# intel/hexl

Measured on NVIDIA H100. Metric: ntt_per_sec_fwd_inv_N65536_q55_batch8192, higher is better.
Workload: dtype u64

## Files before the change

hexl_b200/csrc/ntt_kernels.cuh:

```cuda
#pragma once
#include <algorithm>
#include <atomic>
#include <cstdio>
#include <cstdlib>

#include "internal.h"

namespace hexl_b200 {
namespace {

template <int I>
struct Idx {
  __host__ __device__ constexpr operator int() const { return I; }
};
template <int BEGIN, int END, typename F>
__device__ __forceinline__ void static_for(F&& f) {
  if constexpr (BEGIN < END) {
    f(Idx<BEGIN>{});
    static_for<BEGIN + 1, END>(f);
  }
}

enum : int { kGeneric = 0, kFast = 1, kSmall = 2, kWide = 3 };

template <int MODE>
struct Ar {
  using E = u64;
  using Tw = Twiddle;
};
template <>
struct Ar<kSmall> {
  using E = unsigned;
  using Tw = Twiddle32;
};
constexpr u64 kFastModulusLimit = 1ull << 56;
constexpr u64 kWideModulusLimit = 1ull << 61;
constexpr int kFastProd = 4;
constexpr int kFastBound = 8;

struct Mod {
  u64 q, two_q, four_q, mu;
  unsigned n0, n1;
};

__device__ __forceinline__ unsigned lo32(u64 x) { return (unsigned)x; }
__device__ __forceinline__ unsigned hi32(u64 x) { return (unsigned)(x >> 32); }
__device__ __forceinline__ u64 join(unsigned lo, unsigned hi) {
  u64 r;
  asm("mov.b64 %0, {%1, %2};" : "=l"(r) : "r"(lo), "r"(hi));
  return r;
}
__device__ __forceinline__ void split(u64 x, unsigned& lo, unsigned& hi) {
  asm("mov.b64 {%0, %1}, %2;" : "=r"(lo), "=r"(hi) : "l"(x));
}
__device__ __forceinline__ u64 mul_wide(unsigned a, unsigned b) {
  u64 r;
  asm("mul.wide.u32 %0, %1, %2;" : "=l"(r) : "r"(a), "r"(b));
  return r;
}
__device__ __forceinline__ u64 mad_wide(unsigned a, unsigned b, u64 c) {
  u64 r;
  asm("mad.wide.u32 %0, %1, %2, %3;" : "=l"(r) : "r"(a), "r"(b), "l"(c));
  return r;
}
__device__ __forceinline__ unsigned mad_lo(unsigned a, unsigned b, unsigned c) {
  unsigned r;
  asm("mad.lo.u32 %0, %1, %2, %3;" : "=r"(r) : "r"(a), "r"(b), "r"(c));
  return r;
}

__device__ __forceinline__ Twiddle ld_tw(const Twiddle* p) {
  const ulonglong2 v = __ldg(reinterpret_cast<const ulonglong2*>(p));
  Twiddle t;
  t.w = v.x;
  t.wp = v.y;
  return t;
}
__device__ __forceinline__ Twiddle32 ld_tw(const Twiddle32* p) {
  const uint2 v = __ldg(reinterpret_cast<const uint2*>(p));
  Twiddle32 t;
  t.w = v.x;
  t.wp = v.y;
  return t;
}

__device__ __forceinline__ u64 mulhi_approx(u64 a, u64 b) {
  unsigned a0, a1, b0, b1;
  split(a, a0, a1);
  split(b, b0, b1);
  const u64 hs = (u64)hi32(mul_wide(a1, b0)) + (u64)hi32(mul_wide(a0, b1));
  return mad_wide(a1, b1, hs);
}

__device__ __forceinline__ u64 mad_chain(u64 x, u64 w, u64 Q, const Mod& m) {
  unsigned x0, x1, w0, w1, q0, q1, t0, t1;
  split(x, x0, x1);
  split(w, w0, w1);
  split(Q, q0, q1);
  split(mad_wide(q0, m.n0, mul_wide(x0, w0)), t0, t1);
  t1 = mad_lo(x0, w1, t1);
  t1 = mad_lo(x1, w0, t1);
  t1 = mad_lo(q0, m.n1, t1);
  t1 = mad_lo(q1, m.n0, t1);
  return join(t0, t1);
}

template <int MODE>
__device__ __forceinline__ u64 mul_tw(u64 x, const Twiddle w, const Mod& m) {
  const u64 Q = (MODE == kFast || MODE == kWide) ? mulhi_approx(x, w.wp) : mulhi(x, w.wp);
  return mad_chain(x, w.w, Q, m);
}
__device__ __forceinline__ u64 mul_tw_exact(u64 x, const Twiddle w, const Mod& m) {
  return mad_chain(x, w.w, mulhi(x, w.wp), m);
}

__device__ __forceinline__ u64 barrett_lazy(u64 x, const Mod& m) {
  unsigned q0, q1, t0, t1;
  split(mulhi(x, m.mu), q0, q1);
  split(mad_wide(q0, m.n0, x), t0, t1);
  t1 = mad_lo(q0, m.n1, t1);
  t1 = mad_lo(q1, m.n0, t1);
  return join(t0, t1);
}
__device__ __forceinline__ u64 barrett_lazy_bigq(u64 x, const Mod& m) {
  unsigned x0, x1, s0, s1, t0, t1, Q, dummy;
  split(x, x0, x1);
  const unsigned mu0 = lo32(m.mu);
  split(mul_wide(x1, mu0), s0, s1);
  const unsigned h = hi32(mul_wide(x0, mu0));
  asm("add.cc.u32 %0, %2, %3;\n\taddc.u32 %1, %4, 0;" : "=r"(dummy), "=r"(Q) : "r"(s0), "r"(h), "r"(s1));
  split(mad_wide(Q, m.n0, x), t0, t1);
  return join(t0, mad_lo(Q, m.n1, t1));
}
__device__ __forceinline__ u64 barrett_lazy3_bigq(u64 x, const Mod& m) {
  unsigned x0, x1, t0, t1;
  split(x, x0, x1);
  const unsigned Q = hi32(mul_wide(x1, lo32(m.mu)));
  split(mad_wide(Q, m.n0, x), t0, t1);
  return join(t0, mad_lo(Q, m.n1, t1));
}

__device__ __forceinline__ u64 reduce_any(u64 x, const Mod& m) { return csub_s(barrett_lazy(x, m), m.q); }
__device__ __forceinline__ unsigned reduce_any(unsigned x, const Mod& m) { return x % (unsigned)m.q; }

struct ProdIn {
  const u64* b;
  u64 mu;
  int shift;
};
template <int MODE>
__device__ __forceinline__ u64 prod_lazy(u64 x, u64 y, const Mod& m, u64 pmu, int shift) {
  unsigned x0, x1, y0, y1, q0, q1, t0, t1;
  split(x, x0, x1);
  split(y, y0, y1);
  const u64 t = mul_wide(x0, y0);
  const u64 uu = mad_wide(x0, y1, (u64)hi32(t));
  const u64 vv = mad_wide(x1, y0, (u64)lo32(uu));
  const u64 hi = mad_wide(x1, y1, (u64)hi32(uu) + (u64)hi32(vv));
  const u64 lo = join(lo32(t), lo32(vv));
  const u64 c1 = shift ? ((lo >> shift) | (hi << (64 - shift))) : lo;
  const u64 Q = (MODE == kFast || MODE == kWide) ? mulhi_approx(c1, pmu) : mulhi(c1, pmu);
  split(Q, q0, q1);
  split(mad_wide(q0, m.n0, lo), t0, t1);
  t1 = mad_lo(q0, m.n1, t1);
  t1 = mad_lo(q1, m.n0, t1);
  return join(t0, t1);
}

template <int MODE, typename TW>
__device__ __forceinline__ void fwd_bfly(u64& X, u64& Y, const TW& w, const Mod& m) {
  if (MODE == kFast) {
    const u64 T = mul_tw<kFast>(Y, w, m);
    Y = X + m.four_q - T;
    X = X + T;
  } else if (MODE == kWide) {
    const u64 tx = csub(X, m.four_q);
    const u64 T = mul_tw<kWide>(Y, w, m);
    X = tx + T;
    Y = tx + m.four_q - T;
  } else {
    const u64 tx = csub_s(X, m.two_q);
    const u64 T = mul_tw<kGeneric>(Y, w, m);
    X = tx + T;
    Y = tx + m.two_q - T;
  }
}

template <int MODE, typename TW>
__device__ __forceinline__ void inv_bfly(u64& X, u64& Y, const TW& w, const Mod& m, u64 cq) {
  if (MODE == kFast) {
    const u64 d = X + cq - Y;
    X = X + Y;
    Y = mul_tw<kFast>(d, w, m);
  } else if (MODE == kWide) {
    const u64 s = X + Y;
    const u64 d = X + m.four_q - Y;
    X = csub_s(s, m.four_q);
    Y = mul_tw<kWide>(d, w, m);
  } else {
    const u64 s = X + Y;
    const u64 d = X + m.two_q - Y;
    X = csub_s(s, m.two_q);
    Y = mul_tw<kGeneric>(d, w, m);
  }
}

__device__ __forceinline__ void inv_bfly_last(u64& X, u64& Y, const Twiddle inv_n, const Twiddle inv_n_w,
                                              const Mod& m, u64 cq) {
  const u64 s = X + Y;
  const u64 d = X + cq - Y;
  X = mul_tw_exact(s, inv_n, m);
  Y = mul_tw_exact(d, inv_n_w, m);
}

template <int MODE>
__device__ __forceinline__ u64 fwd_out(u64 v, const Mod& m, int out_mf) {
  if (MODE == kFast) {
    v = barrett_lazy_bigq(v, m);
    return out_mf == 1 ? csub_s(v, m.q) : v;
  }
  if (MODE == kWide) v = csub_s(v, m.four_q);
  return out_mf == 1 ? csub_s(csub_s(v, m.two_q), m.q) : v;
}
__device__ __forceinline__ u64 inv_out(u64 v, const Mod& m, int out_mf) {
  return out_mf == 1 ? csub_s(v, m.q) : v;
}

__device__ __forceinline__ unsigned csub32(unsigned x, unsigned c) { return min(x, x - c); }
__device__ __forceinline__ unsigned mul_tw32(unsigned x, const Twiddle32 w, const Mod& m) {
  const unsigned Q = hi32(mul_wide(x, w.wp));
  return mad_lo(Q, m.n0, x * w.w);
}
template <int MODE, typename TW>
__device__ __forceinline__ void fwd_bfly(unsigned& X, unsigned& Y, const TW& w, const Mod& m) {
  const unsigned two_q = lo32(m.two_q);
  const unsigned tx = csub32(X, two_q);
  const unsigned T = mul_tw32(Y, w, m);
  X = tx + T;
  Y = tx + two_q - T;
}
template <int MODE, typename TW>
__device__ __forceinline__ void inv_bfly(unsigned& X, unsigned& Y, const TW& w, const Mod& m, unsigned) {
  const unsigned two_q = lo32(m.two_q);
  const unsigned s = X + Y;
  const unsigned d = X + two_q - Y;
  X = csub32(s, two_q);
  Y = mul_tw32(d, w, m);
}
__device__ __forceinline__ void inv_bfly_last(unsigned& X, unsigned& Y, const Twiddle32 inv_n,
                                              const Twiddle32 inv_n_w, const Mod& m, unsigned) {
  const unsigned s = X + Y;
  const unsigned d = X + lo32(m.two_q) - Y;
  X = mul_tw32(s, inv_n, m);
  Y = mul_tw32(d, inv_n_w, m);
}
template <int MODE>
__device__ __forceinline__ unsigned fwd_out(unsigned v, const Mod& m, int out_mf) {
  return out_mf == 1 ? csub32(csub32(v, lo32(m.two_q)), lo32(m.q)) : v;
}
__device__ __forceinline__ unsigned inv_out(unsigned v, const Mod& m, int out_mf) {
  return out_mf == 1 ? csub32(v, lo32(m.q)) : v;
}

__host__ __device__ constexpr int inv_slot_bound(int K, int low) {
  if (low == 0) return kFastBound << K;
  int h = 0;
  for (int b = 0; b < K; ++b)
    if (low & (1 << b)) h = b;
  return kFastProd << (K - 1 - h);
}
__host__ __device__ constexpr int inv_stage_cover(int s) { return kFastBound << s; }
template <int MODE>
__device__ __forceinline__ typename Ar<MODE>::E stage_cq(int step, const Mod& m) {
  if (MODE == kFast) return (u64)inv_stage_cover(step) * m.q;
  if (MODE == kWide) return m.four_q;
  return (typename Ar<MODE>::E)m.two_q;
}

template <int K, int NSLOTS, int E = 0>
__device__ __forceinline__ void inv_pass_fixup(u64* v, const Mod& m) {
  if constexpr (E < NSLOTS) {
    if constexpr (inv_slot_bound(K, E & ((1 << K) - 1)) > kFastBound) v[E] = barrett_lazy3_bigq(v[E], m);
    inv_pass_fixup<K, NSLOTS, E + 1>(v, m);
  }
}

template <typename E>
__device__ __forceinline__ unsigned swz(unsigned j) {
  return j ^ ((j >> 4) & (sizeof(E) == 8 ? 15u : 31u));
}
__host__ __device__ constexpr unsigned pad_slot(int e, int lb) { return ((unsigned)e << lb) + (((unsigned)e << lb) >> 4); }
template <typename E>
__host__ __device__ constexpr unsigned row_elems(int logc) {
  return (1u << logc) + (sizeof(E) == 8 ? (1u << logc) >> 4 : 0u);
}

template <int LB>
__device__ __forceinline__ unsigned reg_index(unsigned u, int e) {
  return ((u >> LB) << (LB + 4)) | ((unsigned)e << LB) | (u & ((1u << LB) - 1u));
}

constexpr int kRowTwEntries = 17 * 16;
template <int LOGC, int LB, int HB, int LOB>
struct PassTw {
  static constexpr int kDepth = LOGC - LB - 4;
  static constexpr bool kShared = LOGC >= 8 && (HB - LOB) == 3 && (kDepth == 0 || kDepth == 4);
  static constexpr int kOffset = kDepth == 0 ? 0 : 16;
};

template <int LOGC, typename Tw>
__device__ __forceinline__ void load_row_twiddles(Tw* stab, unsigned tid, unsigned nthreads, u64 base,
                                                  const Tw* __restrict__ tw) {
  for (int idx = tid; idx < kRowTwEntries; idx += nthreads) {
    const int l = idx & 15;
    if (l == 0) continue;
    const u64 root = idx < 16 ? base : (base << 4) + ((idx - 16) >> 4);
    const int s = 31 - __clz(l);
    stab[idx] = ld_tw(tw + (root << s) + (l - (1 << s)));
  }
}

template <int MODE, int LOGC, int LB, int HB, int LOB, bool FWD>
__device__ __forceinline__ void reg_stages(typename Ar<MODE>::E (&v)[16], unsigned u, u64 base,
                                           const typename Ar<MODE>::Tw* __restrict__ tw,
                                           const typename Ar<MODE>::Tw* stab, const Mod& m, bool fold,
                                           typename Ar<MODE>::Tw inv_n, typename Ar<MODE>::Tw inv_n_w) {
  using PT = PassTw<LOGC, LB, HB, LOB>;
  using Tw = typename Ar<MODE>::Tw;
  const Tw* sroot = stab + PT::kOffset + ((u >> LB) << 4);
  static_for<0, HB - LOB + 1>([&](auto STEP) {
    constexpr int step = STEP;
    constexpr int beta = FWD ? HB - step : LOB + step;
    constexpr int eb = beta - LB;
    constexpr int sp = LOGC - 1 - beta;
    const typename Ar<MODE>::E cq = stage_cq<MODE>(step, m);
    auto fetch = [&](int g) {
      if constexpr (PT::kShared)
        return sroot[(8 >> eb) + g];
      else
        return ld_tw(tw + (base << (LOGC - 1 - beta)) + ((u64)(u >> LB) << (LB + 3 - beta)) + g);
    };
    auto groups = [&] {
      Tw wc[8 >> eb];
      if constexpr (FWD) static_for<0, (8 >> eb)>([&](auto G) { constexpr int g = G; wc[g] = fetch(g); });
      static_for<0, (8 >> eb)>([&](auto G) {
        constexpr int g = G;
        Tw wt;
        if constexpr (FWD)
          wt = wc[g];
        else
          wt = fetch(g);
        static_for<0, (1 << eb)>([&](auto L) {
          constexpr int e = (g << (eb + 1)) | L;
          if constexpr (FWD)
            fwd_bfly<MODE>(v[e], v[e | (1 << eb)], wt, m);
          else
            inv_bfly<MODE>(v[e], v[e | (1 << eb)], wt, m, cq);
        });
      });
    };
    if constexpr (!FWD && sp == 0) {
      if (fold) {
        static_for<0, (1 << eb)>([&](auto L) {
          constexpr int l = L;
          inv_bfly_last(v[l], v[l | (1 << eb)], inv_n, inv_n_w, m, cq);
        });
      } else {
        groups();
      }
    } else {
      groups();
    }
  });
  if constexpr (!FWD && MODE == kFast) {
    if (!(fold && LOGC - 1 - HB == 0)) inv_pass_fixup<HB - LOB + 1, 16>(v, m);
  }
}

template <int LB_FROM, int LB_TO, typename E>
__device__ __forceinline__ void smem_exchange(E (&v)[16], E* srow, unsigned u) {
  constexpr bool kWarpLocal = (LB_FROM > LB_TO ? LB_FROM : LB_TO) <= 5;
  if constexpr (sizeof(E) == 8) {
    const unsigned uf = reg_index<LB_FROM>(u, 0), ut = reg_index<LB_TO>(u, 0);
    E* wr = srow + (uf + (uf >> 4));
    const E* rd = srow + (ut + (ut >> 4));
    static_for<0, 16>([&](auto I) { constexpr int e = I; wr[pad_slot(e, LB_FROM)] = v[e]; });
    if (kWarpLocal)
      __syncwarp();
    else
      __syncthreads();
    static_for<0, 16>([&](auto I) { constexpr int e = I; v[e] = rd[pad_slot(e, LB_TO)]; });
  } else {
    static_for<0, 16>([&](auto I) { constexpr int e = I; srow[swz<E>(reg_index<LB_FROM>(u, e))] = v[e]; });
    if (kWarpLocal)
      __syncwarp();
    else
      __syncthreads();
    static_for<0, 16>([&](auto I) { constexpr int e = I; v[e] = srow[swz<E>(reg_index<LB_TO>(u, e))]; });
  }
}

template <int MODE, int LOGC, int PASS>
__device__ __forceinline__ void fwd_passes(typename Ar<MODE>::E (&v)[16], typename Ar<MODE>::E* srow, unsigned u,
                                           u64 base, const typename Ar<MODE>::Tw* tw,
                                           const typename Ar<MODE>::Tw* stab, const Mod& m) {
  using Tw = typename Ar<MODE>::Tw;
  constexpr int PREV_LB = (LOGC - 4 * PASS) > 0 ? (LOGC - 4 * PASS) : 0;
  constexpr int HB = LOGC - 4 * PASS - 1;
  if constexpr (HB >= 0) {
    constexpr int LB = (HB - 3) > 0 ? (HB - 3) : 0;
    smem_exchange<PREV_LB, LB>(v, srow, u);
    reg_stages<MODE, LOGC, LB, HB, LB, true>(v, u, base, tw, stab, m, false, Tw{}, Tw{});
    fwd_passes<MODE, LOGC, PASS + 1>(v, srow, u, base, tw, stab, m);
  }
}

template <int MODE, int LOGC, int PASS>
__device__ __forceinline__ void inv_passes(typename Ar<MODE>::E (&v)[16], typename Ar<MODE>::E* srow, unsigned u,
                                           u64 base, const typename Ar<MODE>::Tw* tw,
                                           const typename Ar<MODE>::Tw* stab, const Mod& m, bool fold,
                                           typename Ar<MODE>::Tw inv_n, typename Ar<MODE>::Tw inv_n_w) {
  constexpr int HB = LOGC - 4 * PASS - 1;
  constexpr int LB = (HB - 3) > 0 ? (HB - 3) : 0;
  reg_stages<MODE, LOGC, LB, HB, LB, false>(v, u, base, tw, stab, m, fold, inv_n, inv_n_w);
  if constexpr (PASS > 0) {
    constexpr int NHB = LOGC - 4 * (PASS - 1) - 1;
    constexpr int NLB = (NHB - 3) > 0 ? (NHB - 3) : 0;
    smem_exchange<LB, NLB>(v, srow, u);
    inv_passes<MODE, LOGC, PASS - 1>(v, srow, u, base, tw, stab, m, fold, inv_n, inv_n_w);
  }
}

constexpr int kRowMinBlocks = 3;
constexpr int kRowMinBlocks512 = 2;
constexpr int kRowMinBlocksSmall = 4;
template <int LOGC, int MODE = kGeneric>
struct RowCfg {
  using E = typename Ar<MODE>::E;
  using Tw = typename Ar<MODE>::Tw;
  static constexpr int C = 1 << LOGC;
  static constexpr int T = C / 16;
  static constexpr int ROWS = T >= 256 ? 1 : 256 / T;
  static constexpr int THREADS = T * ROWS;
  static constexpr int PASSES = (LOGC + 3) / 4;
  static constexpr bool TW_TABLES = LOGC >= 8;
  static constexpr size_t ROW_BYTES = (size_t)row_elems<E>(LOGC) * sizeof(E) + (TW_TABLES ? kRowTwEntries * sizeof(Tw) : 0);
  static constexpr size_t SMEM = (size_t)ROWS * ROW_BYTES;
  static constexpr int MIN_BLOCKS = THREADS <= 256 ? (MODE == kSmall ? kRowMinBlocksSmall : kRowMinBlocks)
                                                   : (THREADS == 512 ? kRowMinBlocks512 : 1);
};

enum : int { kStream = 0, kViaL2 = 1, kSmemRow = 2, kSmemRowPad = 3 };
template <int POLICY>
__device__ __forceinline__ u64 ld_coef(const u64* p) {
  return POLICY == kViaL2 ? __ldcg(p) : __ldcs(p);
}
template <int POLICY>
__device__ __forceinline__ void st_coef(u64* p, u64 v) {
  if (POLICY == kViaL2)
    __stcg(p, v);
  else
    __stcs(p, v);
}

template <int POLICY, typename E>
__device__ __forceinline__ E ld_row(const void* base, unsigned idx) {
  if constexpr (POLICY == kSmemRow)
    return static_cast<const E*>(base)[idx];
  else if constexpr (POLICY == kSmemRowPad)
    return static_cast<const E*>(base)[idx + (idx >> 4)];
  else
    return (E)ld_coef<POLICY>(static_cast<const u64*>(base) + idx);
}
template <int POLICY, typename E>
__device__ __forceinline__ void st_row(void* base, unsigned idx, E v) {
  if constexpr (POLICY == kSmemRow)
    static_cast<E*>(base)[idx] = v;
  else if constexpr (POLICY == kSmemRowPad)
    static_cast<E*>(base)[idx + (idx >> 4)] = v;
  else
    st_coef<POLICY>(static_cast<u64*>(base) + idx, v);
}

struct MirrorList {
  u64* const* p;
  unsigned count;
  u64 off;
};

template <int MODE, int LOGC, int LD, int ST>
__device__ __forceinline__ void row_fwd_body(void* out, const void* in, typename Ar<MODE>::E* srow, unsigned u,
                                             u64 base, const typename Ar<MODE>::Tw* __restrict__ tw, const Mod& m,
                                             int out_mf, bool active, typename Ar<MODE>::Tw* cta_stab = nullptr,
                                             bool reduce_in = false) {
  using E = typename Ar<MODE>::E;
  using Tw = typename Ar<MODE>::Tw;
  E v[16];
  constexpr int LB0 = LOGC - 4;
  Tw* stab = cta_stab ? cta_stab : reinterpret_cast<Tw*>(srow + row_elems<E>(LOGC));
  static_for<0, 16>([&](auto I) { constexpr int e = I; v[e] = ld_row<LD, E>(in, reg_index<LB0>(u, e)); });
  if constexpr (LD < kSmemRow && sizeof(E) == 8) {
    if (reduce_in) {
      static_for<0, 16>([&](auto I) { constexpr int e = I; v[e] = reduce_any(v[e], m); });
    }
  }
  if constexpr (RowCfg<LOGC>::TW_TABLES) {
    if (cta_stab)
      load_row_twiddles<LOGC>(stab, threadIdx.x, blockDim.x, base, tw);
    else
      load_row_twiddles<LOGC>(stab, u, (1u << LOGC) / 16, base, tw);
    __syncthreads();
  }
  reg_stages<MODE, LOGC, LB0, LOGC - 1, LB0, true>(v, u, base, tw, stab, m, false, Tw{}, Tw{});
  fwd_passes<MODE, LOGC, 1>(v, srow, u, base, tw, stab, m);
  static_for<0, 16>([&](auto I) { constexpr int e = I; v[e] = fwd_out<MODE>(v[e], m, out_mf); });
  constexpr int LB_OUT = LB0 < 4 ? LB0 : 4;
  if constexpr (LOGC > 4) smem_exchange<0, LB_OUT>(v, srow, u);
  if (active) {
    static_for<0, 16>([&](auto I) { constexpr int e = I; st_row<ST, E>(out, reg_index<LB_OUT>(u, e), v[e]); });
  }
}

template <int MODE, int LOGC, int LD, int ST>
__device__ __forceinline__ void row_inv_body(void* out, const void* in, typename Ar<MODE>::E* srow, unsigned u,
                                             u64 base, const typename Ar<MODE>::Tw* __restrict__ tw, const Mod& m,
                                             int out_mf, bool fold, typename Ar<MODE>::Tw inv_n,
                                             typename Ar<MODE>::Tw inv_n_w, bool active,
                                             typename Ar<MODE>::Tw* cta_stab = nullptr, const MirrorList* mir = nullptr,
                                             const ProdIn* prod = nullptr) {
  using Cfg = RowCfg<LOGC>;
  using E = typename Ar<MODE>::E;
  using Tw = typename Ar<MODE>::Tw;
  E v[16];
  constexpr int LB0 = LOGC - 4;
  constexpr int LB_IN = LB0 < 4 ? LB0 : 4;
  Tw* stab = cta_stab ? cta_stab : reinterpret_cast<Tw*>(srow + row_elems<E>(LOGC));
  static_for<0, 16>([&](auto I) { constexpr int e = I; v[e] = ld_row<LD, E>(in, reg_index<LB_IN>(u, e)); });
  if constexpr (LD < kSmemRow && sizeof(E) == 8) {
    if (prod) {
      static_for<0, 16>([&](auto I) {
        constexpr int e = I;
        v[e] = prod_lazy<MODE>(v[e], ld_coef<LD>(prod->b + reg_index<LB_IN>(u, e)), m, prod->mu, prod->shift);
      });
    }
  }
  if constexpr (Cfg::TW_TABLES) {
    if (cta_stab)
      load_row_twiddles<LOGC>(stab, threadIdx.x, blockDim.x, base, tw);
    else
      load_row_twiddles<LOGC>(stab, u, (1u << LOGC) / 16, base, tw);
    __syncthreads();
  }
  if constexpr (LOGC > 4) smem_exchange<LB_IN, 0>(v, srow, u);
  inv_passes<MODE, LOGC, Cfg::PASSES - 1>(v, srow, u, base, tw, stab, m, fold, inv_n, inv_n_w);
  if (active) {
    static_for<0, 16>([&](auto I) {
      constexpr int e = I;
      st_row<ST, E>(out, reg_index<LB0>(u, e), fold ? inv_out(v[e], m, out_mf) : v[e]);
    });
    if (mir && fold) {
      for (unsigned p = 0; p < mir->count; ++p) {
        static_for<0, 16>([&](auto I) {
          constexpr int e = I;
          mir->p[p][mir->off + reg_index<LB0>(u, e)] = (u64)inv_out(v[e], m, out_mf);
        });
      }
    }
  }
}

template <int MODE, int LOGC>
__global__ void __launch_bounds__(RowCfg<LOGC, MODE>::THREADS, RowCfg<LOGC, MODE>::MIN_BLOCKS)
    ntt_row_fwd(u64* result, const u64* operand, const typename Ar<MODE>::Tw* __restrict__ tw, const Mod m,
                u64 total_rows, unsigned rows_per_poly, int out_mf) {
  using Cfg = RowCfg<LOGC, MODE>;
  extern __shared__ __align__(16) unsigned char smem[];
  const unsigned row_local = threadIdx.x / Cfg::T, u = threadIdx.x % Cfg::T;
  u64 row = (u64)blockIdx.x * Cfg::ROWS + row_local;
  const bool active = row < total_rows;
  if (!active) row = total_rows - 1;
  const u64 base = (u64)rows_per_poly + (row % rows_per_poly);
  typename Cfg::Tw* cta_stab = nullptr;
  if (MODE == kSmall && Cfg::ROWS > 1 && Cfg::TW_TABLES && rows_per_poly == 1)
    cta_stab = reinterpret_cast<typename Cfg::Tw*>(smem + (size_t)row_elems<typename Cfg::E>(LOGC) * sizeof(typename Cfg::E));
  row_fwd_body<MODE, LOGC, kStream, kStream>(
      result + row * Cfg::C, operand + row * Cfg::C,
      reinterpret_cast<typename Cfg::E*>(smem + (size_t)row_local * Cfg::ROW_BYTES), u, base, tw, m, out_mf, active,
      cta_stab);
}

template <int MODE, int LOGC>
__global__ void __launch_bounds__(RowCfg<LOGC, MODE>::THREADS, RowCfg<LOGC, MODE>::MIN_BLOCKS)
    ntt_row_inv(u64* result, const u64* operand, const typename Ar<MODE>::Tw* __restrict__ tw, const Mod m,
                u64 total_rows, unsigned rows_per_poly, int out_mf, int fold, typename Ar<MODE>::Tw inv_n,
                typename Ar<MODE>::Tw inv_n_w) {
  using Cfg = RowCfg<LOGC, MODE>;
  extern __shared__ __align__(16) unsigned char smem[];
  const unsigned row_local = threadIdx.x / Cfg::T, u = threadIdx.x % Cfg::T;
  u64 row = (u64)blockIdx.x * Cfg::ROWS + row_local;
  const bool active = row < total_rows;
  if (!active) row = total_rows - 1;
  const u64 base = (u64)rows_per_poly + (row % rows_per_poly);
  typename Cfg::Tw* cta_stab = nullptr;
  if (MODE == kSmall && Cfg::ROWS > 1 && Cfg::TW_TABLES && rows_per_poly == 1)
    cta_stab = reinterpret_cast<typename Cfg::Tw*>(smem + (size_t)row_elems<typename Cfg::E>(LOGC) * sizeof(typename Cfg::E));
  row_inv_body<MODE, LOGC, kStream, kStream>(
      result + row * Cfg::C, operand + row * Cfg::C,
      reinterpret_cast<typename Cfg::E*>(smem + (size_t)row_local * Cfg::ROW_BYTES), u, base, tw, m, out_mf,
      fold != 0, inv_n, inv_n_w, active, cta_stab);
}

template <int MODE, int LOGR, bool FWD>
__device__ __forceinline__ void col_stages(typename Ar<MODE>::E (&v)[1 << LOGR], const typename Ar<MODE>::Tw* stw,
                                           const Mod& m, bool root_fold, typename Ar<MODE>::Tw inv_n,
                                           typename Ar<MODE>::Tw inv_n_w) {
  using E = typename Ar<MODE>::E;
  using Tw = typename Ar<MODE>::Tw;
  constexpr int R = 1 << LOGR;
  static_for<0, LOGR>([&](auto STEP) {
    constexpr int step = STEP;
    constexpr int s = FWD ? step : LOGR - 1 - step;
    constexpr int eb = LOGR - 1 - s;
    const E cq = stage_cq<MODE>(step, m);
    auto groups = [&] {
      static_for<0, (1 << s)>([&](auto GI) {
        constexpr int gi = GI;
        const Tw w = stw[(1 << s) + gi];
        static_for<0, (1 << eb)>([&](auto L) {
          constexpr int e = (gi << (eb + 1)) | L;
          if constexpr (FWD)
            fwd_bfly<MODE>(v[e], v[e | (1 << eb)], w, m);
          else
            inv_bfly<MODE>(v[e], v[e | (1 << eb)], w, m, cq);
        });
      });
    };
    if constexpr (!FWD && s == 0) {
      if (root_fold) {
        static_for<0, (1 << eb)>([&](auto L) {
          constexpr int l = L;
          inv_bfly_last(v[l], v[l | (1 << eb)], inv_n, inv_n_w, m, cq);
        });
      } else {
        groups();
      }
    } else {
      groups();
    }
  });
  if constexpr (!FWD && MODE == kFast) {
    if (!root_fold) inv_pass_fixup<LOGR, R>(v, m);
  }
}

template <int MODE, int LOGR, bool FWD, int LD, int ST>
__device__ __forceinline__ void col_body(u64* result, const u64* operand, u64 off, int log_stride,
                                         const typename Ar<MODE>::Tw* stw, const Mod& m, int out_mf, bool root_fold,
                                         typename Ar<MODE>::Tw inv_n, typename Ar<MODE>::Tw inv_n_w,
                                         const MirrorList* mir = nullptr, bool reduce_in = false) {
  using E = typename Ar<MODE>::E;
  constexpr int R = 1 << LOGR;
  E v[R];
  static_for<0, R>([&](auto I) {
    constexpr int e = I;
    v[e] = (E)ld_coef<LD>(operand + off + ((u64)e << log_stride));
  });
  if constexpr (FWD && sizeof(E) == 8) {
    if (reduce_in) {
      static_for<0, R>([&](auto I) { constexpr int e = I; v[e] = reduce_any(v[e], m); });
    }
  }
  col_stages<MODE, LOGR, FWD>(v, stw, m, root_fold, inv_n, inv_n_w);
  const bool final_out = !FWD && root_fold;
  static_for<0, R>([&](auto I) {
    constexpr int e = I;
    st_coef<ST>(result + off + ((u64)e << log_stride), final_out ? inv_out(v[e], m, out_mf) : v[e]);
  });
  if (mir && final_out) {
    for (unsigned p = 0; p < mir->count; ++p) {
      static_for<0, R>([&](auto I) {
        constexpr int e = I;
        mir->p[p][mir->off + off + ((u64)e << log_stride)] = (u64)inv_out(v[e], m, out_mf);
      });
    }
  }
}

template <int MODE, int LOGR, bool FWD>
__global__ void __launch_bounds__(256)
    ntt_col(u64* result, const u64* operand, const typename Ar<MODE>::Tw* __restrict__ tw, const Mod m, int log_n,
            int log_s, u64 total_cols, int out_mf, int fold, typename Ar<MODE>::Tw inv_n,
            typename Ar<MODE>::Tw inv_n_w) {
  constexpr int R = 1 << LOGR;
  __shared__ typename Ar<MODE>::Tw stw[R];
  const int log_cols = log_s - LOGR;
  const u64 g0 = (u64)blockIdx.x * blockDim.x;
  const u64 blk = g0 >> log_cols;
  const u64 blocks_per_poly = 1ull << (log_n - log_s);
  const u64 base = blocks_per_poly + (blk & (blocks_per_poly - 1));
  for (int l = threadIdx.x; l < R; l += blockDim.x) {
    if (l == 0) continue;
    const int s = 31 - __clz(l);
    stw[l] = ld_tw(tw + (base << s) + (l - (1 << s)));
  }
  __syncthreads();
  const u64 g = g0 + threadIdx.x;
  if (g >= total_cols) return;
  const u64 c = g & ((1ull << log_cols) - 1);
  col_body<MODE, LOGR, FWD, kStream, kStream>(result, operand, (blk << log_s) + c, log_cols, stw, m, out_mf,
                                              !FWD && fold && log_s == log_n, inv_n, inv_n_w);
}

__device__ __forceinline__ void cluster_barrier() {
  asm volatile("barrier.cluster.arrive.release.aligned;\n\tbarrier.cluster.wait.acquire.aligned;" ::: "memory");
}

template <int LOGR>
struct FusedCfg {
  static constexpr int LOGC = 12, C = 1 << LOGC, R = 1 << LOGR;
  static constexpr int K = R < 8 ? R : 8;
  static constexpr int THREADS = 256;
  static constexpr int MIN_BLOCKS = LOGR <= 4 ? kRowMinBlocks : 2;
  static constexpr size_t SMEM = RowCfg<LOGC>::ROW_BYTES;
};

template <int MODE, int LOGR>
__global__ void __launch_bounds__(FusedCfg<LOGR>::THREADS, FusedCfg<LOGR>::MIN_BLOCKS)
    ntt_fused_fwd(u64* result, const u64* operand, const typename Ar<MODE>::Tw* __restrict__ tw, const Mod m,
                  int out_mf) {
  using Cfg = FusedCfg<LOGR>;
  using E = typename Ar<MODE>::E;
  using Tw = typename Ar<MODE>::Tw;
  extern __shared__ __align__(16) unsigned char smem_raw[];
  E* smem = reinterpret_cast<E*>(smem_raw);
  __shared__ Tw stw[Cfg::R];
// ... 179 lines not shown
    });
  }
  cluster_barrier();
#pragma unroll 1
  for (int lr = 0; lr < Cfg::RPC; ++lr) {
    const unsigned r = rank + lr * Cfg::K;
    E* row = rows + lr * Cfg::ROW;
    row_fwd_body<MODE, Cfg::LOGC, Cfg::ROW_POLICY, kStream>(result + poly_off + (u64)r * Cfg::C, row,
                                                            Cfg::PAD ? row : xbuf, threadIdx.x, (u64)Cfg::R + r, tw, m,
                                                            out_mf, true, ctab);
    if (lr + 1 < Cfg::RPC) __syncthreads();
  }
}

template <int MODE, int LOGR>
__global__ void __launch_bounds__(DsmemCfg<LOGR, MODE>::THREADS, DsmemCfg<LOGR, MODE>::MIN_BLOCKS)
    ntt_dsmem_inv(u64* result, const u64* operand, const typename Ar<MODE>::Tw* __restrict__ tw, const Mod m,
                  int out_mf, typename Ar<MODE>::Tw inv_n, typename Ar<MODE>::Tw inv_n_w) {
  using Cfg = DsmemCfg<LOGR, MODE>;
  using E = typename Ar<MODE>::E;
  using Tw = typename Ar<MODE>::Tw;
  extern __shared__ __align__(16) unsigned char smem_raw[];
  E* rows = reinterpret_cast<E*>(smem_raw);
  E* xbuf = rows + Cfg::RPC * Cfg::ROW;
  Tw* const ctab = Cfg::PAD ? reinterpret_cast<Tw*>(xbuf) : nullptr;
  __shared__ Tw stw[Cfg::R];
  const unsigned rank = blockIdx.x % Cfg::K;
  const u64 poly_off = (u64)(blockIdx.x / Cfg::K) << (Cfg::LOGC + LOGR);
  for (int l = threadIdx.x; l < Cfg::R; l += Cfg::THREADS)
    if (l) stw[l] = ld_tw(tw + l);
#pragma unroll 1
  for (int lr = 0; lr < Cfg::RPC; ++lr) {
    const unsigned r = rank + lr * Cfg::K;
    E* row = rows + lr * Cfg::ROW;
    row_inv_body<MODE, Cfg::LOGC, kStream, Cfg::ROW_POLICY>(row, operand + poly_off + (u64)r * Cfg::C,
                                                            Cfg::PAD ? row : xbuf, threadIdx.x, (u64)Cfg::R + r, tw, m,
                                                            out_mf, false, inv_n, inv_n_w, true, ctab);
    __syncthreads();
  }
  cluster_barrier();
  unsigned owner_base[Cfg::K];
  static_for<0, Cfg::K>([&](auto I) { constexpr int o = I; owner_base[o] = dsmem_address(rows, o); });
#pragma unroll 1
  for (int c = threadIdx.x; c < Cfg::COLS; c += Cfg::THREADS) {
    const unsigned col = rank * Cfg::COLS + c;
    E v[Cfg::R];
    static_for<0, Cfg::R>([&](auto I) {
      constexpr int e = I;
      v[e] = dsmem_load<E>(owner_base[e % Cfg::K] + ((e / Cfg::K) * Cfg::ROW + Cfg::slot(col)) * (unsigned)sizeof(E));
    });
    col_stages<MODE, LOGR, false>(v, stw, m, true, inv_n, inv_n_w);
    static_for<0, Cfg::R>([&](auto I) {
      constexpr int e = I;
      st_coef<kStream>(result + poly_off + ((u64)e << Cfg::LOGC) + col, inv_out(v[e], m, out_mf));
    });
  }
  cluster_barrier();
}

template <bool FWD>
__global__ void ntt_stage_simple(u64* result, const u64* src, const Twiddle* __restrict__ tw,
                                 const Mod m, int log_n, int s ,
                                 u64 total_bflies, int out_mf, int last, Twiddle inv_n,
                                 Twiddle inv_n_w) {
  const u64 g = (u64)blockIdx.x * blockDim.x + threadIdx.x;
  if (g >= total_bflies) return;
  const int log_t = log_n - 1 - s;
  const u64 half = 1ull << (log_n - 1);
  const u64 poly = g >> (log_n - 1), k = g & (half - 1);
  const u64 i = k >> log_t, jj = k & ((1ull << log_t) - 1);
  const u64 j = (poly << log_n) + (i << (log_t + 1)) + jj;
  u64 X = src[j], Y = src[j + (1ull << log_t)];
  if (FWD) {
    fwd_bfly<kGeneric>(X, Y, ld_tw(tw + (1ull << s) + i), m);
    if (last) {
      X = fwd_out<kGeneric>(X, m, out_mf);
      Y = fwd_out<kGeneric>(Y, m, out_mf);
    }
  } else if (last) {
    inv_bfly_last(X, Y, inv_n, inv_n_w, m, m.two_q);
    X = inv_out(X, m, out_mf);
    Y = inv_out(Y, m, out_mf);
  } else {
    inv_bfly<kGeneric>(X, Y, ld_tw(tw + (1ull << s) + i), m, m.two_q);
  }
  result[j] = X;
  result[j + (1ull << log_t)] = Y;
}


template <auto Kernel>
cudaError_t ensure_dynamic_smem(size_t bytes) {
  if (bytes <= 48 * 1024) return cudaSuccess;
  static std::atomic<unsigned long long> done{0};
  int dev = 0;
  cudaGetDevice(&dev);
  const unsigned long long bit = 1ull << (dev & 63);
  if (done.load(std::memory_order_acquire) & bit) return cudaSuccess;
  const cudaError_t e = cudaFuncSetAttribute(Kernel, cudaFuncAttributeMaxDynamicSharedMemorySize, (int)bytes);
  if (e == cudaSuccess) done.fetch_or(bit, std::memory_order_release);
  return e;
}

template <auto Kernel, typename Cfg, typename... Args>
cudaError_t launch_pipelined(u64 units, cudaStream_t stream, Args... args) {
  static const unsigned lookahead = [] {
    const char* v = std::getenv("HEXL_B200_PIPE_LOOKAHEAD");
    return (unsigned)std::max(1, v ? std::atoi(v) : 16);
  }();
  cudaError_t e = ensure_dynamic_smem<Kernel>(Cfg::SMEM);
  if (e != cudaSuccess) return e;
  int dev = 0, sms = 0;
  cudaGetDevice(&dev);
  cudaDeviceGetAttribute(&sms, cudaDevAttrMultiProcessorCount, dev);
  const u64 items = (units + lookahead) * Cfg::SLOTS;
  const unsigned grid = (unsigned)std::min<u64>((u64)sms * Cfg::MIN_BLOCKS, items);
  unsigned* state = nullptr;
  const size_t bytes = (size_t)(units + 1) * sizeof(unsigned);
  if ((e = scratch_alloc_async(reinterpret_cast<void**>(&state), bytes, stream)) != cudaSuccess) return e;
  if ((e = cudaMemsetAsync(state, 0, bytes, stream)) == cudaSuccess) {
    Kernel<<<grid, Cfg::THREADS, Cfg::SMEM, stream>>>(args..., (unsigned)units, lookahead, state, state + 1);
    count_launch();
    e = cudaGetLastError();
  }
  scratch_free_async(state, stream);
  return e;
}

inline int pick_row_log(int log_n) { return log_n <= 13 ? log_n : 12; }

inline int pick_mode(u64 q) {
  if (q < kSmallModulusLimit) return kSmall;
  if (q < kFastModulusLimit && q >= (1ull << 32)) return kFast;
  return (q >= kFastModulusLimit && q < kWideModulusLimit) ? kWide : kGeneric;
}

template <int MODE>
struct Tab {
  static const Twiddle* fwd(const NttDeviceTables& t) { return t.fwd; }
  static const Twiddle* inv(const NttDeviceTables& t) { return t.inv; }
  static Twiddle inv_n(const NttDeviceTables& t) { return t.inv_n; }
  static Twiddle inv_n_w(const NttDeviceTables& t) { return t.inv_n_w; }
};
template <>
struct Tab<kSmall> {
  static const Twiddle32* fwd(const NttDeviceTables& t) { return t.fwd32; }
  static const Twiddle32* inv(const NttDeviceTables& t) { return t.inv32; }
  static Twiddle32 inv_n(const NttDeviceTables& t) { return t.inv_n32; }
  static Twiddle32 inv_n_w(const NttDeviceTables& t) { return t.inv_n_w32; }
};

__host__ __device__ inline Mod make_mod(u64 q, u64 mu) {
  Mod m;
  m.q = q;
  m.two_q = q << 1;
  m.four_q = q << 2;
  m.mu = mu;
  const u64 negq = 0 - q;
  m.n0 = (unsigned)negq;
  m.n1 = (unsigned)(negq >> 32);
  return m;
}
inline Mod make_mod(const NttDeviceTables& t) { return make_mod(t.q, t.mu); }

inline int plan_col_passes(int top_stages, int out[8]) {
  if (top_stages <= 0) return 0;
  const int passes = (top_stages + 4) / 5;
  int left = top_stages;
  for (int p = 0; p < passes; ++p) {
    out[p] = (left + (passes - p) - 1) / (passes - p);
    left -= out[p];
  }
  return passes;
}


}
}
```

hexl_b200/csrc/ntt_multi.cu:

```cuda
#include "ntt_kernels.cuh"

namespace hexl_b200 {
namespace {

__device__ __forceinline__ NttDeviceParams load_params(const NttMulti& multi, u64 poly) {
  return *multi.p[poly / multi.group];
}

template <int MODE, int LOGC, bool FWD, bool MUL = false>
__global__ void __launch_bounds__(RowCfg<LOGC, MODE>::THREADS, RowCfg<LOGC, MODE>::MIN_BLOCKS)
    ntt_row_multi(u64* result, const u64* operand, const __grid_constant__ NttMulti multi, u64 total_rows,
                  unsigned rows_per_poly, int out_mf, int fold, unsigned gather) {
  using Cfg = RowCfg<LOGC, MODE>;
  extern __shared__ __align__(16) unsigned char smem[];
  const unsigned row_local = threadIdx.x / Cfg::T, u = threadIdx.x % Cfg::T;
  u64 row = (u64)blockIdx.x * Cfg::ROWS + row_local;
  const bool active = row < total_rows;
  if (!active) row = total_rows - 1;
  const NttDeviceParams P = load_params(multi, row / rows_per_poly);
  const Mod m = make_mod(P.q, P.mu);
  const u64 base = (u64)rows_per_poly + (row % rows_per_poly);
  typename Cfg::E* srow = reinterpret_cast<typename Cfg::E*>(smem + (size_t)row_local * Cfg::ROW_BYTES);
  if (FWD) {
    const u64 poly = row / rows_per_poly;
// ... 72 lines not shown
      __syncthreads();
    }
    const u64 poly_off = (u64)poly << (Cfg::LOGC + LOGR);
    if (!producer) {
      if (threadIdx.x == 0)
        while (ld_acquire_gpu(done + poly) < (unsigned)Cfg::CT) __nanosleep(100);
      __syncthreads();
    }
    if (producer) {
      col_body<MODE, LOGR, true, kStream, kViaL2>(result, operand, poly_off + j * Cfg::THREADS + threadIdx.x, Cfg::LOGC,
                                                  stw, m, out_mf, false, Twiddle{}, Twiddle{});
    } else {
      const unsigned r = j - Cfg::CT;
      u64* row = result + poly_off + (u64)r * Cfg::C;
      row_fwd_body<MODE, Cfg::LOGC, kViaL2, kStream>(row, row, smem, threadIdx.x, (u64)Cfg::R + r, P.fwd, m, out_mf,
                                                     true);
    }
    if (producer) {
      __syncthreads();
      if (threadIdx.x == 0) red_release_gpu(done + poly, 1u);
    }
  }
}

template <bool FWD, int LOGN>
__global__ void ntt_tiny_multi(u64* result, const u64* operand, const __grid_constant__ NttMulti multi, u64 units,
                               int out_mf) {
  const u64 unit = (u64)blockIdx.x * blockDim.x + threadIdx.x;
  if (unit >= units) return;
  const NttDeviceParams P = *multi.p[unit / multi.group];
  const Mod m = make_mod(P.q, P.mu);
  constexpr int n = 1 << LOGN;
  u64 v[n];
  const u64 src_unit = (FWD && multi.gather) ? unit % multi.gather : unit;
  static_for<0, n>([&](auto I) {
    constexpr int e = I;
    v[e] = operand[src_unit * n + e];
    if (FWD && multi.gather) v[e] %= P.q;
    if (!FWD && multi.mul) v[e] = prod_lazy<kGeneric>(v[e], multi.mul[unit * n + e], m, P.prod_mu, P.prod_shift);
  });
  static_for<0, LOGN>([&](auto K) {
    constexpr int k = K;
    constexpr int s = FWD ? k : LOGN - 1 - k;
    constexpr int t = n >> (s + 1);
    static_for<0, (1 << s)>([&](auto I) {
      constexpr int i = I;
      static_for<0, t>([&](auto J) {
        constexpr int j = J;
        u64& X = v[2 * i * t + j];
        u64& Y = v[2 * i * t + j + t];
        if constexpr (FWD)
          fwd_bfly<kGeneric>(X, Y, P.fwd[(1 << s) + i], m);
        else if constexpr (s == 0)
          inv_bfly_last(X, Y, P.inv_n, P.inv_n_w, m, m.two_q);
        else
          inv_bfly<kGeneric>(X, Y, P.inv[(1 << s) + i], m, m.two_q);
      });
    });
  });
  static_for<0, n>([&](auto I) {
    constexpr int e = I;
    result[unit * n + e] = FWD ? fwd_out<kGeneric>(v[e], m, out_mf) : inv_out(v[e], m, out_mf);
  });
  if (!FWD)
    for (unsigned p = 0; p < multi.mirrors; ++p)
      static_for<0, n>([&](auto I) {
        constexpr int e = I;
        multi.mirror[p][unit * n + e] = inv_out(v[e], m, out_mf);
      });
}

template <int MODE, int LOGC>
cudaError_t launch_row_multi(bool fwd, const NttMulti& multi, int log_n, u64* result, const u64* operand, u64 units,
                             int out_mf, int fold, cudaStream_t stream, unsigned gather = 0) {
  using Cfg = RowCfg<LOGC, MODE>;
  const unsigned rows_per_poly = 1u << (log_n - LOGC);
  const u64 total_rows = units * rows_per_poly;
  const unsigned grid = (unsigned)((total_rows + Cfg::ROWS - 1) / Cfg::ROWS);
  if (fwd) {
    if (cudaError_t e = ensure_dynamic_smem<ntt_row_multi<MODE, LOGC, true>>(Cfg::SMEM)) return e;
    ntt_row_multi<MODE, LOGC, true><<<grid, Cfg::THREADS, Cfg::SMEM, stream>>>(result, operand, multi, total_rows,
                                                                               rows_per_poly, out_mf, fold, gather);
  } else if (multi.mul) {
    if (cudaError_t e = ensure_dynamic_smem<ntt_row_multi<MODE, LOGC, false, true>>(Cfg::SMEM)) return e;
    ntt_row_multi<MODE, LOGC, false, true><<<grid, Cfg::THREADS, Cfg::SMEM, stream>>>(result, operand, multi, total_rows,
                                                                                      rows_per_poly, out_mf, fold, 0u);
  } else {
    if (cudaError_t e = ensure_dynamic_smem<ntt_row_multi<MODE, LOGC, false>>(Cfg::SMEM)) return e;
    ntt_row_multi<MODE, LOGC, false><<<grid, Cfg::THREADS, Cfg::SMEM, stream>>>(result, operand, multi, total_rows,
                                                                                rows_per_poly, out_mf, fold, 0u);
  }
  count_launch();
  return cudaGetLastError();
}

template <int MODE>
cudaError_t launch_row_multi_dyn(int log_c, bool fwd, const NttMulti& multi, int log_n, u64* result,
                                 const u64* operand, u64 units, int out_mf, int fold, cudaStream_t stream,
                                 unsigned gather = 0) {
  switch (log_c) {
#define ROW_CASE(L) \
  case L: return launch_row_multi<MODE, L>(fwd, multi, log_n, result, operand, units, out_mf, fold, stream, gather);
    ROW_CASE(4) ROW_CASE(5) ROW_CASE(6) ROW_CASE(7) ROW_CASE(8) ROW_CASE(9) ROW_CASE(10)
    ROW_CASE(11) ROW_CASE(12) ROW_CASE(13)
#undef ROW_CASE
  }
  return cudaErrorInvalidValue;
}

template <int MODE, int LOGR>
cudaError_t launch_col_multi(bool fwd, const NttMulti& multi, int log_n, u64* result, const u64* operand, u64 units,
                             int log_s, int out_mf, int fold, cudaStream_t stream, unsigned gather = 0) {
  const u64 total_cols = (units << log_n) >> LOGR;
  const u64 cols_per_block = 1ull << (log_s - LOGR);
  const unsigned threads = (unsigned)(cols_per_block < 256 ? cols_per_block : 256);
  const unsigned grid = (unsigned)((total_cols + threads - 1) / threads);
  if (fwd)
    ntt_col_multi<MODE, LOGR, true><<<grid, threads, 0, stream>>>(result, operand, multi, log_n, log_s, total_cols,
                                                                  out_mf, fold, gather);
  else
    ntt_col_multi<MODE, LOGR, false><<<grid, threads, 0, stream>>>(result, operand, multi, log_n, log_s, total_cols,
// ... 81 lines not shown
```

Measured before the change: 1.376 million.

## Rebalance NTT modular arithmetic across ALU pipes and cheapen inverse fixups

Adds an opaque zero field to Mod so some butterfly additions are forced onto a different integer instruction path instead of the IMAD pipe. The Barrett reduction is split into mul_wide plus a 64-bit add rather than a fused mad_wide. Fast and wide modes now use lazy mul_tw in the last inverse butterfly, with a final csub on output. Small inverse fixup bounds are handled with conditional subtractions instead of a full Barrett reduction. Row load and store index math is hoisted so only the base is computed per thread. Correctness depends on the new lazy bounds staying within range.

```diff
diff --git a/hexl_b200/csrc/ntt_kernels.cuh b/hexl_b200/csrc/ntt_kernels.cuh
--- a/hexl_b200/csrc/ntt_kernels.cuh
+++ b/hexl_b200/csrc/ntt_kernels.cuh
@@ -41,6 +41,7 @@
 struct Mod {
   u64 q, two_q, four_q, mu;
   unsigned n0, n1;
+  unsigned zero;
 };
 
 __device__ __forceinline__ unsigned lo32(u64 x) { return (unsigned)x; }
@@ -68,6 +69,8 @@
   asm("mad.lo.u32 %0, %1, %2, %3;" : "=r"(r) : "r"(a), "r"(b), "r"(c));
   return r;
 }
+
+__device__ __forceinline__ u64 add_alu(u64 a, u64 b, const Mod& m) { return a + b + m.zero; }
 
 __device__ __forceinline__ Twiddle ld_tw(const Twiddle* p) {
   const ulonglong2 v = __ldg(reinterpret_cast<const ulonglong2*>(p));
@@ -133,11 +136,13 @@
   return join(t0, mad_lo(Q, m.n1, t1));
 }
 __device__ __forceinline__ u64 barrett_lazy3_bigq(u64 x, const Mod& m) {
-  unsigned x0, x1, t0, t1;
+  unsigned x0, x1, p0, p1;
   split(x, x0, x1);
   const unsigned Q = hi32(mul_wide(x1, lo32(m.mu)));
-  split(mad_wide(Q, m.n0, x), t0, t1);
-  return join(t0, mad_lo(Q, m.n1, t1));
+  split(mul_wide(Q, m.n0), p0, p1);
+  const unsigned qn1 = Q * m.n1;
+  const u64 s = x + join(p0, p1);
+  return join(lo32(s), hi32(s) + qn1);
 }
 
 __device__ __forceinline__ u64 reduce_any(u64 x, const Mod& m) { return csub_s(barrett_lazy(x, m), m.q); }
@@ -172,11 +177,11 @@
   if (MODE == kFast) {
     const u64 T = mul_tw<kFast>(Y, w, m);
     Y = X + m.four_q - T;
-    X = X + T;
+    X = add_alu(X, T, m);
   } else if (MODE == kWide) {
     const u64 tx = csub(X, m.four_q);
     const u64 T = mul_tw<kWide>(Y, w, m);
-    X = tx + T;
+    X = add_alu(tx, T, m);
     Y = tx + m.four_q - T;
   } else {
     const u64 tx = csub_s(X, m.two_q);
@@ -190,10 +195,10 @@
 __device__ __forceinline__ void inv_bfly(u64& X, u64& Y, const TW& w, const Mod& m, u64 cq) {
   if (MODE == kFast) {
     const u64 d = X + cq - Y;
-    X = X + Y;
+    X = add_alu(X, Y, m);
     Y = mul_tw<kFast>(d, w, m);
   } else if (MODE == kWide) {
-    const u64 s = X + Y;
+    const u64 s = add_alu(X, Y, m);
     const u64 d = X + m.four_q - Y;
     X = csub_s(s, m.four_q);
     Y = mul_tw<kWide>(d, w, m);
@@ -205,24 +210,29 @@
   }
 }
 
+template <int MODE>
 __device__ __forceinline__ void inv_bfly_last(u64& X, u64& Y, const Twiddle inv_n, const Twiddle inv_n_w,
                                               const Mod& m, u64 cq) {
-  const u64 s = X + Y;
+  const u64 s = add_alu(X, Y, m);
   const u64 d = X + cq - Y;
-  X = mul_tw_exact(s, inv_n, m);
-  Y = mul_tw_exact(d, inv_n_w, m);
+  if (MODE == kFast || MODE == kWide) {
+    X = mul_tw<MODE>(s, inv_n, m);
+    Y = mul_tw<MODE>(d, inv_n_w, m);
+  } else {
+    X = mul_tw_exact(s, inv_n, m);
+    Y = mul_tw_exact(d, inv_n_w, m);
+  }
 }
 
 template <int MODE>
 __device__ __forceinline__ u64 fwd_out(u64 v, const Mod& m, int out_mf) {
-  if (MODE == kFast) {
-    v = barrett_lazy_bigq(v, m);
-    return out_mf == 1 ? csub_s(v, m.q) : v;
-  }
+  if (MODE == kFast) v = barrett_lazy3_bigq(v, m);
   if (MODE == kWide) v = csub_s(v, m.four_q);
   return out_mf == 1 ? csub_s(csub_s(v, m.two_q), m.q) : v;
 }
+template <int MODE>
 __device__ __forceinline__ u64 inv_out(u64 v, const Mod& m, int out_mf) {
+  if (MODE == kFast || MODE == kWide) v = csub_s(v, m.two_q);
   return out_mf == 1 ? csub_s(v, m.q) : v;
 }
 
@@ -247,6 +257,7 @@
   X = csub32(s, two_q);
   Y = mul_tw32(d, w, m);
 }
+template <int MODE>
 __device__ __forceinline__ void inv_bfly_last(unsigned& X, unsigned& Y, const Twiddle32 inv_n,
                                               const Twiddle32 inv_n_w, const Mod& m, unsigned) {
   const unsigned s = X + Y;
@@ -258,6 +269,7 @@
 __device__ __forceinline__ unsigned fwd_out(unsigned v, const Mod& m, int out_mf) {
   return out_mf == 1 ? csub32(csub32(v, lo32(m.two_q)), lo32(m.q)) : v;
 }
+template <int MODE>
 __device__ __forceinline__ unsigned inv_out(unsigned v, const Mod& m, int out_mf) {
   return out_mf == 1 ? csub32(v, lo32(m.q)) : v;
 }
@@ -277,10 +289,17 @@
   return (typename Ar<MODE>::E)m.two_q;
 }
 
+constexpr int kFastFixupCsub = 32;
 template <int K, int NSLOTS, int E = 0>
 __device__ __forceinline__ void inv_pass_fixup(u64* v, const Mod& m) {
   if constexpr (E < NSLOTS) {
-    if constexpr (inv_slot_bound(K, E & ((1 << K) - 1)) > kFastBound) v[E] = barrett_lazy3_bigq(v[E], m);
+    constexpr int bound = inv_slot_bound(K, E & ((1 << K) - 1));
+    if constexpr (bound > kFastFixupCsub) {
+      v[E] = barrett_lazy3_bigq(v[E], m);
+    } else {
+      if constexpr (bound > 2 * kFastBound) v[E] = csub_s(v[E], m.four_q << 2);
+      if constexpr (bound > kFastBound) v[E] = csub_s(v[E], m.four_q << 1);
+    }
     inv_pass_fixup<K, NSLOTS, E + 1>(v, m);
   }
 }
@@ -363,7 +382,7 @@
       if (fold) {
         static_for<0, (1 << eb)>([&](auto L) {
           constexpr int l = L;
-          inv_bfly_last(v[l], v[l | (1 << eb)], inv_n, inv_n_w, m, cq);
+          inv_bfly_last<MODE>(v[l], v[l | (1 << eb)], inv_n, inv_n_w, m, cq);
         });
       } else {
         groups();
@@ -464,22 +483,24 @@
 }
 
 template <int POLICY, typename E>
-__device__ __forceinline__ E ld_row(const void* base, unsigned idx) {
+__device__ __forceinline__ E ld_row(const void* base, unsigned u0, unsigned off) {
+  const unsigned idx = u0 + off;
   if constexpr (POLICY == kSmemRow)
     return static_cast<const E*>(base)[idx];
   else if constexpr (POLICY == kSmemRowPad)
     return static_cast<const E*>(base)[idx + (idx >> 4)];
   else
-    return (E)ld_coef<POLICY>(static_cast<const u64*>(base) + idx);
+    return (E)ld_coef<POLICY>(static_cast<const u64*>(base) + u0 + off);
 }
 template <int POLICY, typename E>
-__device__ __forceinline__ void st_row(void* base, unsigned idx, E v) {
+__device__ __forceinline__ void st_row(void* base, unsigned u0, unsigned off, E v) {
+  const unsigned idx = u0 + off;
   if constexpr (POLICY == kSmemRow)
     static_cast<E*>(base)[idx] = v;
   else if constexpr (POLICY == kSmemRowPad)
     static_cast<E*>(base)[idx + (idx >> 4)] = v;
   else
-    st_coef<POLICY>(static_cast<u64*>(base) + idx, v);
+    st_coef<POLICY>(static_cast<u64*>(base) + u0 + off, v);
 }
 
 struct MirrorList {
@@ -498,7 +519,8 @@
   E v[16];
   constexpr int LB0 = LOGC - 4;
   Tw* stab = cta_stab ? cta_stab : reinterpret_cast<Tw*>(srow + row_elems<E>(LOGC));
-  static_for<0, 16>([&](auto I) { constexpr int e = I; v[e] = ld_row<LD, E>(in, reg_index<LB0>(u, e)); });
+  const unsigned u_in = reg_index<LB0>(u, 0);
+  static_for<0, 16>([&](auto I) { constexpr int e = I; v[e] = ld_row<LD, E>(in, u_in, e << LB0); });
   if constexpr (LD < kSmemRow && sizeof(E) == 8) {
     if (reduce_in) {
       static_for<0, 16>([&](auto I) { constexpr int e = I; v[e] = reduce_any(v[e], m); });
@@ -517,7 +539,8 @@
   constexpr int LB_OUT = LB0 < 4 ? LB0 : 4;
   if constexpr (LOGC > 4) smem_exchange<0, LB_OUT>(v, srow, u);
   if (active) {
-    static_for<0, 16>([&](auto I) { constexpr int e = I; st_row<ST, E>(out, reg_index<LB_OUT>(u, e), v[e]); });
+    const unsigned u_out = reg_index<LB_OUT>(u, 0);
+    static_for<0, 16>([&](auto I) { constexpr int e = I; st_row<ST, E>(out, u_out, e << LB_OUT, v[e]); });
   }
 }
 
@@ -535,7 +558,8 @@
   constexpr int LB0 = LOGC - 4;
   constexpr int LB_IN = LB0 < 4 ? LB0 : 4;
   Tw* stab = cta_stab ? cta_stab : reinterpret_cast<Tw*>(srow + row_elems<E>(LOGC));
-  static_for<0, 16>([&](auto I) { constexpr int e = I; v[e] = ld_row<LD, E>(in, reg_index<LB_IN>(u, e)); });
+  const unsigned u_in = reg_index<LB_IN>(u, 0);
+  static_for<0, 16>([&](auto I) { constexpr int e = I; v[e] = ld_row<LD, E>(in, u_in, e << LB_IN); });
   if constexpr (LD < kSmemRow && sizeof(E) == 8) {
     if (prod) {
       static_for<0, 16>([&](auto I) {
@@ -556,13 +580,13 @@
   if (active) {
     static_for<0, 16>([&](auto I) {
       constexpr int e = I;
-      st_row<ST, E>(out, reg_index<LB0>(u, e), fold ? inv_out(v[e], m, out_mf) : v[e]);
+      st_row<ST, E>(out, reg_index<LB0>(u, 0), e << LB0, fold ? inv_out<MODE>(v[e], m, out_mf) : v[e]);
     });
     if (mir && fold) {
       for (unsigned p = 0; p < mir->count; ++p) {
         static_for<0, 16>([&](auto I) {
           constexpr int e = I;
-          mir->p[p][mir->off + reg_index<LB0>(u, e)] = (u64)inv_out(v[e], m, out_mf);
+          mir->p[p][mir->off + reg_index<LB0>(u, e)] = (u64)inv_out<MODE>(v[e], m, out_mf);
         });
       }
     }
@@ -639,7 +663,7 @@
       if (root_fold) {
         static_for<0, (1 << eb)>([&](auto L) {
           constexpr int l = L;
-          inv_bfly_last(v[l], v[l | (1 << eb)], inv_n, inv_n_w, m, cq);
+          inv_bfly_last<MODE>(v[l], v[l | (1 << eb)], inv_n, inv_n_w, m, cq);
         });
       } else {
         groups();
@@ -674,13 +698,13 @@
   const bool final_out = !FWD && root_fold;
   static_for<0, R>([&](auto I) {
     constexpr int e = I;
-    st_coef<ST>(result + off + ((u64)e << log_stride), final_out ? inv_out(v[e], m, out_mf) : v[e]);
+    st_coef<ST>(result + off + ((u64)e << log_stride), final_out ? inv_out<MODE>(v[e], m, out_mf) : v[e]);
   });
   if (mir && final_out) {
     for (unsigned p = 0; p < mir->count; ++p) {
       static_for<0, R>([&](auto I) {
         constexpr int e = I;
-        mir->p[p][mir->off + off + ((u64)e << log_stride)] = (u64)inv_out(v[e], m, out_mf);
+        mir->p[p][mir->off + off + ((u64)e << log_stride)] = (u64)inv_out<MODE>(v[e], m, out_mf);
       });
     }
   }
@@ -966,7 +990,7 @@
     col_stages<MODE, LOGR, false>(v, stw, m, true, inv_n, inv_n_w);
     static_for<0, Cfg::R>([&](auto I) {
       constexpr int e = I;
-      st_coef<kStream>(result + poly_off + ((u64)e << Cfg::LOGC) + col, inv_out(v[e], m, out_mf));
+      st_coef<kStream>(result + poly_off + ((u64)e << Cfg::LOGC) + col, inv_out<MODE>(v[e], m, out_mf));
     });
   }
   cluster_barrier();
@@ -992,9 +1016,9 @@
       Y = fwd_out<kGeneric>(Y, m, out_mf);
     }
   } else if (last) {
-    inv_bfly_last(X, Y, inv_n, inv_n_w, m, m.two_q);
-    X = inv_out(X, m, out_mf);
-    Y = inv_out(Y, m, out_mf);
+    inv_bfly_last<kGeneric>(X, Y, inv_n, inv_n_w, m, m.two_q);
+    X = inv_out<kGeneric>(X, m, out_mf);
+    Y = inv_out<kGeneric>(Y, m, out_mf);
   } else {
     inv_bfly<kGeneric>(X, Y, ld_tw(tw + (1ull << s) + i), m, m.two_q);
   }
@@ -1073,6 +1097,7 @@
   const u64 negq = 0 - q;
   m.n0 = (unsigned)negq;
   m.n1 = (unsigned)(negq >> 32);
+  m.zero = 0;
   return m;
 }
 inline Mod make_mod(const NttDeviceTables& t) { return make_mod(t.q, t.mu); }
diff --git a/hexl_b200/csrc/ntt_multi.cu b/hexl_b200/csrc/ntt_multi.cu
--- a/hexl_b200/csrc/ntt_multi.cu
+++ b/hexl_b200/csrc/ntt_multi.cu
@@ -148,7 +148,7 @@
         if constexpr (FWD)
           fwd_bfly<kGeneric>(X, Y, P.fwd[(1 << s) + i], m);
         else if constexpr (s == 0)
-          inv_bfly_last(X, Y, P.inv_n, P.inv_n_w, m, m.two_q);
+          inv_bfly_last<kGeneric>(X, Y, P.inv_n, P.inv_n_w, m, m.two_q);
         else
           inv_bfly<kGeneric>(X, Y, P.inv[(1 << s) + i], m, m.two_q);
       });
@@ -156,13 +156,13 @@
   });
   static_for<0, n>([&](auto I) {
     constexpr int e = I;
-    result[unit * n + e] = FWD ? fwd_out<kGeneric>(v[e], m, out_mf) : inv_out(v[e], m, out_mf);
+    result[unit * n + e] = FWD ? fwd_out<kGeneric>(v[e], m, out_mf) : inv_out<kGeneric>(v[e], m, out_mf);
   });
   if (!FWD)
     for (unsigned p = 0; p < multi.mirrors; ++p)
       static_for<0, n>([&](auto I) {
         constexpr int e = I;
-        multi.mirror[p][unit * n + e] = inv_out(v[e], m, out_mf);
+        multi.mirror[p][unit * n + e] = inv_out<kGeneric>(v[e], m, out_mf);
       });
 }
 
```

Result: faster. 1.419 million (median of 6 runs) (+3.1%).
